# Mamo1031/Multimodal-MTRSSM

Measured on AMD Instinct MI355X. Metric: seq-steps/s (BxT) MoPoE-MRSSM train step, higher is better.
Workload: dtype bf16x2-split, fp32 accumulate; 1 GPU; BASELINE configs[1]: MoPoE-MRSSM train step, B=64/GPU T=50 deter=200 stoch=30, vision 1x64x64 + audio 1x128x32 + action 4; global_batch=64, seq_len=50, parallelism=dp1, hidden=200, embed=256, categoricals_x_classes=6x5, residual_blocks=3, activation=ELU, optimizer=AdamW lr 1e-3 + clip 10 (fused HIP), params=4151600, streams=1, launch=eager (host enqueues every launch), backend=none, rccl_ranks=0, collective_ranks=0, noise=uniforms keyed by global batch row (parallel.GlobalRowNoise)

## Files before the change

multimodal_mtrssm_amd/csrc/mrssm_cluster.hip:

```cpp
#include "scan_common.h"

namespace mtrssm {

void set_error(const char* fmt, ...);
void set_last_kernel(const char* name);
int device_cu_count();

constexpr int kClu = 4;
constexpr int kCluThreads = 256;
constexpr unsigned kSpinLimit = 1u << 22;

__device__ unsigned long long* g_cluster_prof = nullptr;
#define MTRSSM_CLU_STAMP(i)                                                                                  \
  do {                                                                                                       \
    if (prof && t >= 8 && t < 12) prof[(t - 8) * 16 + (i)] = __builtin_readcyclecounter();                   \
  } while (0)

__device__ __forceinline__ void granule_store(unsigned long long* p, unsigned epoch, float v) {
  __hip_atomic_store(p, ((unsigned long long)epoch << 32) | (unsigned long long)__float_as_uint(v), __ATOMIC_RELAXED,
                     __HIP_MEMORY_SCOPE_AGENT);
}

template <int NJ>
__device__ __forceinline__ bool wave_gather(const unsigned long long* g, float* dst, int total, unsigned epoch, int lane) {
  unsigned done = 0;
  const unsigned full = (1u << NJ) - 1u;
#pragma unroll
  for (int j = 0; j < NJ; ++j)
    if (lane + 64 * j >= total) done |= 1u << j;
  for (unsigned spins = 0;; ++spins) {
#pragma unroll
    for (int j = 0; j < NJ; ++j) {
      if (!(done & (1u << j))) {
        const unsigned long long x = __hip_atomic_load(g + lane + 64 * j, __ATOMIC_RELAXED, __HIP_MEMORY_SCOPE_AGENT);
        if ((unsigned)(x >> 32) == epoch) {
          dst[lane + 64 * j] = __uint_as_float((unsigned)x);
          done |= 1u << j;
        }
      }
    }
    if (__all(done == full)) return true;
    if (spins > kSpinLimit) return false;
    __builtin_amdgcn_s_sleep(1);
  }
}

template <int DH, int NP, int PPT, bool MASKED>
__global__ __launch_bounds__(kCluThreads) void mrssm_fwd_cluster_kernel(const MtrssmMrssmDims dm, const MtrssmMrssmClusterWeights w,
                                                                        const MtrssmMrssmFwdIO io, unsigned long long* __restrict__ gran,
                                                                        int* __restrict__ status, int nclusters) {
  extern __shared__ __attribute__((aligned(16))) float lds[];
  constexpr int D = DH, H = DH;
  constexpr int UD = D / kClu, UH = H / kClu;
  constexpr int NG = 3 * UD, NH = 3 * UH;
  constexpr int KP = DH / NP;
  constexpr int NPIECE = 2 * NG * NP;
  static_assert(KP % 4 == 0 && DH % NP == 0, "pieces are whole float4 runs");
  static_assert(PPT * kCluThreads >= NPIECE, "every piece has a thread");
  const int K = dm.K, C = dm.C, S = K * C, T = dm.T, act = dm.act;
  const int tid = threadIdx.x, lane = tid & (kWave - 1), wave = tid / kWave;
  const int blk = blockIdx.x;
  const int member = (blk >> 3) & (kClu - 1);
  const int cluster = (blk & 7) + 8 * (blk >> 5);
  if (cluster >= nclusters) return;

  int o = 0;
  auto take = [&](int n) { const int r = o; o += (n + 3) & ~3; return r; };
  const int Ls = take(S), Lh1 = take(DH), Ld0 = take(DH), Ld1 = take(DH), Lhd = take(3 * 64);
  const int Llp = take(S), Lla = take(S), Llv = take(S), Lmx = take(S);
  const int Lpart = take(kClu * 3 * S);
  const int Lred = take(NPIECE > NH * NP ? NPIECE : NH * NP);
  const int Lw1 = take(S * H);
  const int Lwh = take(D * NH);
  const int Lbl = take(3 * S);
  const int Lu = take(2 * 64);
  const int Lflag = take(4);
  (void)o;
  int* abort_flag = reinterpret_cast<int*>(lds + Lflag);

  float wreg[PPT][KP];
  int xsel[PPT];
#pragma unroll
  for (int i = 0; i < PPT; ++i) {
    const int pc = tid * PPT + i;
    const int pcc = pc < NPIECE ? pc : NPIECE - 1;
    const int col = pcc / NP, part = pcc - col * NP;
    const bool is_h = col >= NG;
    const int og = is_h ? col - NG : col;
    const int gcol = (og / UD) * D + member * UD + (og % UD);
    const float* src = (is_h ? w.whh_t : w.wf_t) + (size_t)(part * KP) * 3 * D + gcol;
    xsel[i] = (is_h ? 1 : 0) | (part * KP) << 1;
#pragma unroll
    for (int k = 0; k < KP; ++k) wreg[i][k] = src[(size_t)k * 3 * D];
  }
  float wrow[64];
  {
    const bool roleL = tid < 3 * S;
    const int which = roleL ? tid / S : 0, srow = roleL ? tid - which * S : 0;
    const float* rowsrc = (which == 0 ? w.w4 : (which == 1 ? w.wa2 : w.wv2)) + (size_t)srow * H + member * UH;
#pragma unroll
    for (int k = 0; k < 64; ++k) wrow[k] = k < UH ? rowsrc[k] : 0.f;
  }
  for (int idx = tid; idx < S * H; idx += kCluThreads) lds[Lw1 + idx] = w.w1s_t[idx];
  for (int idx = tid; idx < D * NH; idx += kCluThreads) {
    const int k = idx / NH, oh = idx - k * NH;
    lds[Lwh + idx] = w.wh1_t[(size_t)k * 3 * H + (oh / UH) * H + member * UH + (oh % UH)];
  }
  for (int i = tid; i < 3 * 64; i += kCluThreads) lds[Lhd + i] = 0.f;
  for (int i = tid; i < 3 * S; i += kCluThreads) {
    const int which = i / S, s2 = i - which * S;
    lds[Lbl + i] = (which == 0 ? w.b4 : (which == 1 ? w.ba2 : w.bv2))[s2];
  }
  float bias_g[6] = {0.f, 0.f, 0.f, 0.f, 0.f, 0.f};
  if (tid < UD) {
#pragma unroll
    for (int g = 0; g < 3; ++g) {
      bias_g[g] = w.bf[g * D + member * UD + tid];
      bias_g[3 + g] = w.bhh[g * D + member * UD + tid];
    }
  }
  const float bias_h = (tid < UH) ? w.b3[member * UH + tid] : 0.f;
  if (tid == 0) *abort_flag = 0;

  const int slotsD = UD, slotsL = 3 * S;
  const int per_parity = kClu * (slotsD + slotsL);
  unsigned long long* gbase = gran + (size_t)cluster * 2 * per_parity;
  unsigned epoch = 0;
  unsigned long long* prof = (blockIdx.x == 0 && tid == 0) ? g_cluster_prof : nullptr;

  for (int row = cluster; row < dm.B; row += nclusters) {
    int cur = Ld0, nxt = Ld1;
    lds_barrier();
    for (int i = tid; i < D; i += kCluThreads) lds[cur + i] = io.deter0[(size_t)row * D + i];
    for (int i = tid; i < S; i += kCluThreads) lds[Ls + i] = io.stoch0[(size_t)row * S + i];
    lds_barrier();

    auto load_inputs = [&](size_t q, float& xa_r, float& pa_r, float& up_r, float& ur_r, int& code_r) {
      code_r = modality_code<MASKED>(io.modality, q);
      xa_r = tid < H ? io.xa[q * H + tid] : 0.f;
      pa_r = 0.f;
      if (tid >= UH && tid < NH) {
        const int which = tid / UH, u = tid - which * UH;
        pa_r = (which == 1 ? io.pa : io.pv)[q * H + member * UH + u];
      }
      up_r = (wave == 3 && lane < K) ? io.u_post[q * K + lane] : 0.f;
      ur_r = (wave == 3 && lane < K && io.u_prior) ? io.u_prior[q * K + lane] : 0.f;
    };
    float xa_n, pav_n, up_n, ur_n;
    int code_n;
    load_inputs((size_t)row * T, xa_n, pav_n, up_n, ur_n, code_n);

    for (int t = 0; t < T; ++t) {
      const size_t bt = (size_t)row * T + t;
      unsigned long long* gpar = gbase + (size_t)(t & 1) * per_parity;
      const float xa_v = xa_n, pav = pav_n;
      const int code = code_n;
      if (wave == 3 && lane < K) { lds[Lu + lane] = up_n; lds[Lu + 64 + lane] = ur_n; }
      if (t + 1 < T) load_inputs(bt + 1, xa_n, pav_n, up_n, ur_n, code_n);

      MTRSSM_CLU_STAMP(0);
      if (tid < H) {
        const float* wc = lds + Lw1 + tid;
        float a0 = xa_v, a1 = 0.f, a2 = 0.f, a3 = 0.f;
        int k = 0;
        for (; k + 8 <= S; k += 8) {
          float wv[8], sv[8];
#pragma unroll
          for (int i = 0; i < 8; ++i) { wv[i] = wc[(size_t)(k + i) * H]; sv[i] = lds[Ls + k + i]; }
          a0 = fmaf(wv[0], sv[0], a0); a1 = fmaf(wv[1], sv[1], a1); a2 = fmaf(wv[2], sv[2], a2); a3 = fmaf(wv[3], sv[3], a3);
          a0 = fmaf(wv[4], sv[4], a0); a1 = fmaf(wv[5], sv[5], a1); a2 = fmaf(wv[6], sv[6], a2); a3 = fmaf(wv[7], sv[7], a3);
        }
        for (; k < S; ++k) a0 = fmaf(wc[(size_t)k * H], lds[Ls + k], a0);
        const float h = act_fwd((a0 + a1) + (a2 + a3), act);
        lds[Lh1 + tid] = h;
        if (member == 0 && io.sv_h1) io.sv_h1[bt * H + tid] = h;
      }
      lds_barrier();

      MTRSSM_CLU_STAMP(1);
#pragma unroll
      for (int i = 0; i < PPT; ++i) {
        const float* xv = lds + ((xsel[i] & 1) ? cur : Lh1) + (xsel[i] >> 1);
        float a0 = 0.f, a1 = 0.f, a2 = 0.f, a3 = 0.f;
#pragma unroll
        for (int k = 0; k < KP; k += 4) {
          const float4 x = *reinterpret_cast<const float4*>(xv + k);
          a0 = fmaf(wreg[i][k], x.x, a0);
          a1 = fmaf(wreg[i][k + 1], x.y, a1);
          a2 = fmaf(wreg[i][k + 2], x.z, a2);
          a3 = fmaf(wreg[i][k + 3], x.w, a3);
        }
        if (tid * PPT + i < NPIECE) lds[Lred + tid * PPT + i] = (a0 + a1) + (a2 + a3);
      }
      lds_barrier();

      MTRSSM_CLU_STAMP(2);
      ++epoch;
      if (tid < UD) {
        float gs[6];
#pragma unroll
        for (int g = 0; g < 6; ++g) {
          const float* pr = lds + Lred + ((g < 3 ? g : g - 3) * UD + tid + (g < 3 ? 0 : NG)) * NP;
          float a = bias_g[g];
#pragma unroll
          for (int q = 0; q < NP; ++q) a += pr[q];
          gs[g] = a;
        }
        const float rg = __fdividef(1.f, 1.f + __expf(-(gs[3] + gs[0])));
        const float zg = __fdividef(1.f, 1.f + __expf(-(gs[4] + gs[1])));
        const float ng = 1.f - __fdividef(2.f, __expf(2.f * (gs[2] + gs[5] * rg)) + 1.f);
        const int unit = member * UD + tid;
        const float dnew = (lds[cur + unit] - ng) * zg + ng;
        lds[nxt + unit] = dnew;
        granule_store(gpar + (size_t)member * slotsD + tid, epoch, dnew);
        io.deter[bt * D + unit] = dnew;
        if (io.sv_gates) {
          float* gsv = io.sv_gates + bt * 4 * D;
          gsv[unit] = rg; gsv[D + unit] = zg; gsv[2 * D + unit] = ng; gsv[3 * D + unit] = gs[5];
        }
      }
      if (wave == 3) {
        const bool ok = wave_gather<4>(gpar, lds + nxt, D, epoch, lane);
        if (!ok && lane == 0) { *abort_flag = 1; atomicExch(status, 1 + 2 * t); }
      }
      lds_barrier();
// ... 35 lines not shown
      if (tid < 3 * S) {
        const float* hv = lds + Lhd + (tid / S) * 64;
        float p0 = 0.f, p1 = 0.f;
#pragma unroll
        for (int u = 0; u < 64; u += 4) {
          const float4 x = *reinterpret_cast<const float4*>(hv + u);
          p0 = fmaf(wrow[u], x.x, p0);
          p1 = fmaf(wrow[u + 1], x.y, p1);
          p0 = fmaf(wrow[u + 2], x.z, p0);
          p1 = fmaf(wrow[u + 3], x.w, p1);
        }
        const float p = p0 + p1;
        lds[Lpart + member * 3 * S + tid] = p;
        granule_store(gl + (size_t)member * slotsL + tid, epoch, p);
      }
      if (wave == 3) {
        const bool ok = wave_gather<6>(gl, lds + Lpart, kClu * 3 * S, epoch, lane);
        if (!ok && lane == 0) { *abort_flag = 1; atomicExch(status, 2 + 2 * t); }
      }
      lds_barrier();
      if (*abort_flag) return;

      MTRSSM_CLU_STAMP(5);
      if (wave == 3) {
        const bool writer = member == 0;
        for (int i = lane; i < 3 * S; i += kWave) {
          const int which = i / S, s2 = i - which * S;
          float v = lds[Lbl + i];
#pragma unroll
          for (int m2 = 0; m2 < kClu; ++m2) v += lds[Lpart + m2 * 3 * S + i];
          lds[(which == 0 ? Llp : (which == 1 ? Lla : Llv)) + s2] = v;
        }
        wave_mopoe_mix_masked<true, MASKED>(lds + Lla, lds + Llv, lds + Llp, lds + Lmx, S, lane, code);
        for (int s = lane; s < S; s += kWave) {
          if (writer) {
            io.prior_logits[bt * S + s] = lds[Llp + s];
            io.post_logits[bt * S + s] = lds[Lmx + s];
            if (io.sv_la) { io.sv_la[bt * S + s] = lds[Lla + s]; io.sv_lv[bt * S + s] = lds[Llv + s]; }
          }
        }
        float kl = C <= 8 ? cat_block_fwd_fast8(lds + Lmx, lds + Llp, K, C, lane, lds + Lu, io.u_prior ? lds + Lu + 64 : nullptr, lds + Ls,
                                                io.post_stoch + bt * S, io.prior_stoch ? io.prior_stoch + bt * S : nullptr, writer)
                          : cat_block_fwd<true, true>(lds + Lmx, lds + Llp, K, C, lane, lds + Lu, io.u_prior ? lds + Lu + 64 : nullptr, lds + Ls,
                                                      io.post_stoch + bt * S, io.prior_stoch ? io.prior_stoch + bt * S : nullptr, writer);
        if (io.kl) {
          kl = wave_sum(kl);
          if (lane == 0 && writer) io.kl[bt] = kl;
        }
      }
      lds_barrier();
      MTRSSM_CLU_STAMP(7);
      const int tmp = cur; cur = nxt; nxt = tmp;
    }
  }
}

template <int NJ, typename Map>
__device__ __forceinline__ bool wave_gather_map(int total, unsigned epoch, int lane, Map map) {
  unsigned done = 0;
  const unsigned full = (1u << NJ) - 1u;
#pragma unroll
  for (int j = 0; j < NJ; ++j)
    if (lane + 64 * j >= total) done |= 1u << j;
  for (unsigned spins = 0;; ++spins) {
#pragma unroll
    for (int j = 0; j < NJ; ++j) {
      if (!(done & (1u << j))) {
        const unsigned long long* slot;
        float* dst;
        map(lane + 64 * j, slot, dst);
        const unsigned long long x = __hip_atomic_load(slot, __ATOMIC_RELAXED, __HIP_MEMORY_SCOPE_AGENT);
// ... 25 lines not shown
  static_assert(NG % NPB == 0 && KPB % 2 == 0, "row pieces are whole float2 runs");
  static_assert(PPT * kCluThreads >= NPIECE, "every row piece has a thread");
  const int K = dm.K, C = dm.C, S = K * C, T = dm.T, act = dm.act;
  const int tid = threadIdx.x, lane = tid & (kWave - 1), wave = tid / kWave;
  const int blk = blockIdx.x;
  const int member = (blk >> 3) & (kClu - 1);
  const int cluster = (blk & 7) + 8 * (blk >> 5);
  if (cluster >= nclusters) return;

  int o = 0;
  auto take = [&](int n) { const int r = o; o += (n + 3) & ~3; return r; };
  const int Lla = take(S), Llv = take(S), Lmx = take(S), Llp = take(S), Ldmx = take(S), Ldlp = take(S), Ldla = take(S), Ldlv = take(S);
  const int Lgps = take(S), Lcs = take(S);
  const int Lhd = take(NHP), Ldzh = take(NHP);
  const int Lgate = take(4 * UD), Ldprev = take(UD), Lgd = take(UD), Lcd = take(UD);
  const int Ldg = take(2 * NG);
  const int Lh1 = take(DH), Ldz1 = take(DH);
  const int Lpdd = take(kClu * UD);
  const int Lpcd = take(kClu * UD), Lpdh = take(kClu * DH);
  const int Lred = take(NPIECE > DH ? NPIECE : DH);
  const int Lred2 = take(W1P * 64 > 3 * 64 ? W1P * 64 : 3 * 64);
  const int Lwh = take(D * NHP);
  const int Lw2 = take(32 * NHP);
  const int Lflag = take(4);
  (void)o;
  int* abort_flag = reinterpret_cast<int*>(lds + Lflag);
  float* gk_lds = lds + Lflag + 1;

  float wreg[PPT][KPB];
#pragma unroll
  for (int i = 0; i < PPT; ++i) {
    const int pc = tid * PPT + i;
    const int pcc = pc < NPIECE ? pc : NPIECE - 1;
    const int rowi = pcc / NPB, part = pcc - rowi * NPB;
    const bool is_f = rowi >= DH;
    const float* src = (is_f ? w.wf_t : w.whh_t) + (size_t)(is_f ? rowi - DH : rowi) * 3 * D;
#pragma unroll
    for (int k = 0; k < KPB; ++k) {
      const int og = part * KPB + k;
      wreg[i][k] = src[(og / UD) * D + member * UD + (og % UD)];
    }
  }
  for (int idx = tid; idx < 32 * NHP; idx += kCluThreads) {
    const int s2 = idx / NHP, j = idx - s2 * NHP;
    float v = 0.f;
    if (s2 < S && j < NH) {
// ... 1 lines not shown
      v = (which == 0 ? w.w4 : (which == 1 ? w.wa2 : w.wv2))[(size_t)s2 * H + member * UH + u];
    }
    lds[Lw2 + idx] = v;
  }
  float w1r[KW1];
  {
    const int srow = tid / W1P < S ? tid / W1P : 0, part = tid % W1P;
#pragma unroll
    for (int k = 0; k < KW1; ++k) {
      const int kk = part * KW1 + k;
      w1r[k] = w.w1s_t[(size_t)srow * H + (kk < H ? kk : H - 1)];
    }
  }
  for (int idx = tid; idx < D * NHP; idx += kCluThreads) {
    const int k = idx / NHP, oh = idx - k * NHP;
    lds[Lwh + idx] = oh < NH ? w.wh1_t[(size_t)k * 3 * H + (oh / UH) * H + member * UH + (oh % UH)] : 0.f;
  }
  for (int i = tid; i < NHP; i += kCluThreads) { lds[Lhd + i] = 0.f; lds[Ldzh + i] = 0.f; }
  if (tid == 0) *abort_flag = 0;

  const int per_parity = kClu * 3 * D;
  unsigned long long* gbase = gran + (size_t)cluster * 2 * per_parity;
  unsigned epoch = 0;

  for (int row = cluster; row < dm.B; row += nclusters) {
    lds_barrier();
    for (int i = tid; i < UD; i += kCluThreads) lds[Lcd + i] = 0.f;
    for (int i = tid; i < S; i += kCluThreads) lds[Lcs + i] = 0.f;
    lds_barrier();

    float r0 = 0.f, r1 = 0.f, r2 = 0.f, r3 = 0.f, r4 = 0.f;
    int code_n = kModBoth;
    auto stage_load = [&](int tt) {
      const size_t q = (size_t)row * T + tt;
      code_n = modality_code<MASKED>(io.modality, q);
      if (tid < 4 * S) {
        const int which = tid / S, s2 = tid - which * S;
        const float* src = which == 0 ? io.sv_la : (which == 1 ? io.sv_lv : (which == 2 ? io.post_logits : io.prior_logits));
        r0 = src[q * S + s2];
      }
      if (tid < NH) {
        const int which = tid / UH, u = tid - which * UH;
        r1 = io.sv_heads[q * 3 * H + which * H + member * UH + u];
      } else if (tid < NH + S) {
        r1 = io.g_post_stoch ? io.g_post_stoch[q * S + (tid - NH)] : 0.f;
      }
// ... 10 lines not shown
      } else if (tid >= 64 && tid < 64 + UD) {
        r4 = io.g_deter ? io.g_deter[q * D + member * UD + (tid - 64)] : 0.f;
      }
    };
    auto stage_store = [&]() {
      if (tid < 4 * S) {
        const int which = tid / S, s2 = tid - which * S;
        lds[(which == 0 ? Lla : (which == 1 ? Llv : (which == 2 ? Lmx : Llp))) + s2] = r0;
      }
      if (tid < NH) lds[Lhd + tid] = r1;
      else if (tid < NH + S) lds[Lgps + tid - NH] = r1;
      if (tid < 4 * UD) lds[Lgate + tid] = r2;
      else if (tid == 4 * UD) *gk_lds = r2;
      if (tid < H) lds[Lh1 + tid] = r3;
      if (tid < UD) lds[Ldprev + tid] = r4;
      else if (tid >= 64 && tid < 64 + UD) lds[Lgd + tid - 64] = r4;
    };
    stage_load(T - 1);

    for (int t = T - 1; t >= 0; --t) {
      const size_t bt = (size_t)row * T + t;
      unsigned long long* gpar = gbase + (size_t)(t & 1) * per_parity;

      stage_store();
      const int code = code_n;
      if (t > 0) stage_load(t - 1);
      lds_barrier();

      if (wave == 3) {
        if (C <= 8)
          cat_block_bwd_fast8(lds + Lmx, lds + Llp, K, C, lane, lds + Lgps, lds + Lcs, io.g_prior_stoch ? io.g_prior_stoch + bt * S : nullptr,
                              io.g_post_logits ? io.g_post_logits + bt * S : nullptr, io.g_prior_logits ? io.g_prior_logits + bt * S : nullptr,
                              *gk_lds, dm.kl_w_post, dm.kl_w_prior, lds + Ldmx, lds + Ldlp);
        else
          cat_block_bwd<true>(lds + Lmx, lds + Llp, K, C, lane, lds + Lgps, lds + Lcs, io.g_prior_stoch ? io.g_prior_stoch + bt * S : nullptr,
                              io.g_post_logits ? io.g_post_logits + bt * S : nullptr, io.g_prior_logits ? io.g_prior_logits + bt * S : nullptr,
                              *gk_lds, dm.kl_w_post, dm.kl_w_prior, lds + Ldmx, lds + Ldlp);
        wave_mopoe_mix_bwd_masked<true, MASKED>(lds + Lla, lds + Llv, lds + Lmx, lds + Ldmx, lds + Ldla, lds + Ldlv, lds + Ldlp, S, lane,
                                                code);
        if (member == 0) {
          for (int s2 = lane; s2 < S; s2 += kWave) {
            io.d_la[bt * S + s2] = lds[Ldla + s2];
            io.d_lv[bt * S + s2] = lds[Ldlv + s2];
            io.d_lp[bt * S + s2] = lds[Ldlp + s2];
          }
        }
      }
      lds_barrier();

      if (tid < NH) {
        const int which = tid / UH;
        const float* dl = lds + (which == 0 ? Ldlp : (which == 1 ? Ldla : Ldlv));
        const float* wc2 = lds + Lw2 + tid;
        float a0 = 0.f, a1 = 0.f;
#pragma unroll
        for (int s2 = 0; s2 < 32; s2 += 2) {
          a0 = fmaf(wc2[s2 * NHP], s2 < S ? dl[s2] : 0.f, a0);
          a1 = fmaf(wc2[(s2 + 1) * NHP], s2 + 1 < S ? dl[s2 + 1] : 0.f, a1);
        }
        const float g = (a0 + a1) * act_grad_from_out(lds[Lhd + tid], act);
        lds[Ldzh + tid] = g;
        const int u = tid - which * UH;
        io.d_zh[bt * 3 * H + which * H + member * UH + u] = g;
      }
      lds_barrier();

      ++epoch;
      if (tid < D) {
        const float* wr = lds + Lwh + (size_t)tid * NHP;
        const float* dz = lds + Ldzh;
        float p0 = 0.f, p1 = 0.f, p2 = 0.f, p3 = 0.f;
#pragma unroll
        for (int j = 0; j < NHP; j += 4) {
          const float4 a = *reinterpret_cast<const float4*>(wr + j);
          const float4 b = *reinterpret_cast<const float4*>(dz + j);
          p0 = fmaf(a.x, b.x, p0); p1 = fmaf(a.y, b.y, p1); p2 = fmaf(a.z, b.z, p2); p3 = fmaf(a.w, b.w, p3);
        }
        granule_store(gpar + (size_t)member * D + tid, epoch, (p0 + p1) + (p2 + p3));
      }
      if (wave == 3) {
        const bool ok = wave_gather_map<4>(kClu * UD, epoch, lane, [&](int i, const unsigned long long*& slot, float*& dst) {
          const int m2 = i / UD, u = i - m2 * UD;
          slot = gpar + (size_t)m2 * D + member * UD + u;
          dst = lds + Lpdd + i;
        });
        if (!ok && lane == 0) { *abort_flag = 1; atomicExch(status, 1 + 2 * t); }
      }
      lds_barrier();
      if (*abort_flag) return;

      if (tid < UD) {
        float dd = lds[Lgd + tid] + lds[Lcd + tid];
#pragma unroll
        for (int m2 = 0; m2 < kClu; ++m2) dd += lds[Lpdd + m2 * UD + tid];
        const float rg = lds[Lgate + tid], zg = lds[Lgate + UD + tid], ng = lds[Lgate + 2 * UD + tid], ghn = lds[Lgate + 3 * UD + tid];
        const float dprev = lds[Ldprev + tid];
        const float dn = dd * (1.f - zg);
        const float dz = dd * (dprev - ng);
        const float dn_pre = dn * (1.f - ng * ng);
        const float dr = dn_pre * ghn;
        const float dr_pre = dr * rg * (1.f - rg);
        const float dz_pre = dz * zg * (1.f - zg);
        lds[Lcd + tid] = dd * zg;
        lds[Ldg + tid] = dr_pre; lds[Ldg + UD + tid] = dz_pre; lds[Ldg + 2 * UD + tid] = dn_pre;
        lds[Ldg + NG + tid] = dr_pre; lds[Ldg + NG + UD + tid] = dz_pre; lds[Ldg + NG + 2 * UD + tid] = dn_pre * rg;
        const int unit = member * UD + tid;
        float* gi = io.d_gi + bt * 3 * D;
        float* gh = io.d_gh + bt * 3 * D;
        gi[unit] = dr_pre; gi[D + unit] = dz_pre; gi[2 * D + unit] = dn_pre;
        gh[unit] = dr_pre; gh[D + unit] = dz_pre; gh[2 * D + unit] = dn_pre * rg;
      }
      lds_barrier();

#pragma unroll
      for (int i = 0; i < PPT; ++i) {
        const int pc = tid * PPT + i;
        const int pcc = pc < NPIECE ? pc : NPIECE - 1;
        const int rowi = pcc / NPB, part = pcc - rowi * NPB;
        const float* xv = lds + Ldg + (rowi >= DH ? 0 : NG) + part * KPB;
        float a0 = 0.f, a1 = 0.f;
#pragma unroll
        for (int k = 0; k < KPB; k += 2) {
          const float2 x = *reinterpret_cast<const float2*>(xv + k);
          a0 = fmaf(wreg[i][k], x.x, a0);
          a1 = fmaf(wreg[i][k + 1], x.y, a1);
        }
        if (pc < NPIECE) lds[Lred + pc] = a0 + a1;
      }
      lds_barrier();
      ++epoch;
      unsigned long long* g2 = gpar + (size_t)kClu * D;
      for (int r2 = tid; r2 < 2 * DH; r2 += kCluThreads) {
        float a = 0.f;
#pragma unroll
        for (int q = 0; q < NPB; ++q) a += lds[Lred + r2 * NPB + q];
        granule_store(g2 + (size_t)member * 2 * D + r2, epoch, a);
      }
      if (wave >= 1) {
        bool ok;
        if (wave == 1) {
          ok = wave_gather_map<4>(kClu * UD, epoch, lane, [&](int i, const unsigned long long*& slot, float*& dst) {
            const int m2 = i / UD, u = i - m2 * UD;
            slot = g2 + (size_t)m2 * 2 * D + member * UD + u;
            dst = lds + Lpcd + i;
          });
        } else {
          const int mb = (wave - 2) * 2;
          ok = wave_gather_map<(2 * DH + 63) / 64>(2 * DH, epoch, lane, [&](int i, const unsigned long long*& slot, float*& dst) {
            const int m2 = mb + i / DH, k = i % DH;
            slot = g2 + (size_t)m2 * 2 * D + D + k;
            dst = lds + Lpdh + m2 * DH + k;
          });
        }
        if (!ok && lane == 0) { *abort_flag = 1; atomicExch(status, 2 + 2 * t); }
      }
      lds_barrier();
      if (*abort_flag) return;

      if (tid < UD) {
        float a = lds[Lcd + tid];
#pragma unroll
        for (int m2 = 0; m2 < kClu; ++m2) a += lds[Lpcd + m2 * UD + tid];
        lds[Lcd + tid] = a;
      }
      if (tid < H) {
        float a = 0.f;
#pragma unroll
        for (int m2 = 0; m2 < kClu; ++m2) a += lds[Lpdh + m2 * DH + tid];
        const float g = a * act_grad_from_out(lds[Lh1 + tid], act);
        lds[Ldz1 + tid] = g;
        if (member == 0) io.d_z1[bt * H + tid] = g;
      }
      lds_barrier();
      {
        const int srow = tid / W1P, part = tid % W1P;
        if (srow < S) {
          float a0 = 0.f;
#pragma unroll
          for (int k = 0; k < KW1; ++k) {
            const int kk = part * KW1 + k;
            a0 = fmaf(w1r[k], kk < H ? lds[Ldz1 + kk] : 0.f, a0);
          }
          lds[Lred2 + srow * W1P + part] = a0;
        }
      }
      lds_barrier();
      if (tid < S) {
        float a = 0.f;
#pragma unroll
        for (int q = 0; q < W1P; ++q) a += lds[Lred2 + tid * W1P + q];
        lds[Lcs + tid] = a;
      }
      lds_barrier();
    }
    if (tid < UD) io.g_deter0[(size_t)row * D + member * UD + tid] = lds[Lcd + tid];
    if (member == 0 && tid < S) io.g_stoch0[(size_t)row * S + tid] = lds[Lcs + tid];
  }
}

static int cluster_npb(int DH) { return (DH == 200 || DH == 128) ? 3 : 1; }

static size_t cluster_bwd_lds_floats(int DH, int S) {
  const int UD = DH / kClu, NG = 3 * UD, NH = NG, NHP = (NH + 3) & ~3, NPB = cluster_npb(DH), NPIECE = 2 * DH * NPB;
  size_t o = 0;
  auto take = [&](size_t n) { o += (n + 3) & ~(size_t)3; };
  for (int i = 0; i < 10; ++i) take(S);
  take(NHP); take(NHP);
  take((size_t)4 * UD); take(UD); take(UD); take(UD);
  take((size_t)2 * NG);
  take(DH); take(DH);
  take((size_t)kClu * UD);
  take((size_t)kClu * UD); take((size_t)kClu * DH);
  take((size_t)(NPIECE > DH ? NPIECE : DH));
  take((size_t)(8 * 64));
  take((size_t)DH * NHP);
  take((size_t)32 * NHP);
  take(4);
  return o;
}

size_t mrssm_cluster_bwd_workspace_bytes(const MtrssmMrssmDims* d) {
  if (!d || d->B <= 0 || d->D <= 0) return 0;
  const int nclusters = d->B < 64 ? d->B : 64;
  return 16 + (size_t)nclusters * 2 * (size_t)kClu * 3 * d->D * sizeof(unsigned long long);
}

int mrssm_cluster_supported(const MtrssmMrssmDims* d);

int mrssm_bwd_cluster_launch(const MtrssmMrssmDims* d, const MtrssmMrssmClusterWeights* w, const MtrssmMrssmBwdIO* io, void* workspace,
                             size_t workspace_bytes, hipStream_t stream) {
  if (!mrssm_cluster_supported(d) || d->K * d->C > 32) {
    set_error("mrssm_rollout_bwd_cluster: dims outside the cluster kernel's regime (ask mtrssm_mrssm_cluster_supported first; S <= 32)");
    return MTRSSM_EINVAL;
  }
  if (!w || !io || !workspace || !w->w1s_t || !w->wf_t || !w->whh_t || !w->wh1_t || !w->w4 || !w->wa2 || !w->wv2 || !io->deter0 ||
      !io->deter || !io->prior_logits || !io->post_logits || !io->sv_h1 || !io->sv_gates || !io->sv_heads || !io->sv_la || !io->sv_lv ||
      !io->g_deter0 || !io->g_stoch0 || !io->d_z1 || !io->d_gi || !io->d_gh || !io->d_zh || !io->d_lp || !io->d_la || !io->d_lv) {
    set_error("mrssm_rollout_bwd_cluster: null required pointer");
    return MTRSSM_EINVAL;
// ... 32 lines not shown
#undef MTRSSM_CLUB_LAUNCH
#undef MTRSSM_CLUB_LAUNCH_M
  e = hipGetLastError();
  if (e != hipSuccess) { set_error("cluster backward scan launch failed: %s", hipGetErrorString(e)); return MTRSSM_ELAUNCH; }
  return MTRSSM_OK;
}

int debug_set_cluster_profile(void* buf) {
  unsigned long long* p = static_cast<unsigned long long*>(buf);
  return hipMemcpyToSymbol(HIP_SYMBOL(g_cluster_prof), &p, sizeof(p)) == hipSuccess ? MTRSSM_OK : MTRSSM_ELAUNCH;
}

static int cluster_kw(int D, int H) { return D > H ? D : H; }

static int cluster_np(int DH) { return DH == 200 ? 5 : (DH == 128 ? 4 : (DH == 64 ? 2 : 1)); }

static size_t cluster_lds_floats(int D, int H, int S) {
  const int UD = D / kClu, UH = H / kClu, NG = 3 * UD, NH = 3 * UH, KW = cluster_kw(D, H), NP = cluster_np(KW);
  size_t o = 0;
  auto take = [&](size_t n) { o += (n + 3) & ~(size_t)3; };
  take(S); take(KW); take(KW); take(KW); take(3 * 64);
  take(S); take(S); take(S); take(S);
  take((size_t)kClu * 3 * S);
  take((size_t)(2 * NG * NP > NH * NP ? 2 * NG * NP : NH * NP));
  take((size_t)S * H);
  take((size_t)D * NH);
  take((size_t)3 * S);
  take(2 * 64);
  take(4);
  return o;
}

size_t mrssm_cluster_workspace_bytes(const MtrssmMrssmDims* d) {
  if (!d || d->B <= 0 || d->D <= 0 || d->K <= 0 || d->C <= 0) return 0;
  const int nclusters = d->B < 64 ? d->B : 64;
  const size_t per_parity = (size_t)kClu * (d->D / kClu + 3 * d->K * d->C);
  return 16 + (size_t)nclusters * 2 * per_parity * sizeof(unsigned long long);
}

int mrssm_cluster_supported(const MtrssmMrssmDims* d) {
  if (!d || d->B <= 0 || d->T <= 0 || d->D <= 0 || d->H <= 0 || d->K <= 0 || d->C <= 0 || !d->post) return 0;
  const int S = d->K * d->C, D = d->D, H = d->H;
  if (D != H || (D != 32 && D != 64 && D != 128 && D != 200)) return 0;
  if (3 * S > kCluThreads || H / kClu > 64 || 3 * H / kClu > kCluThreads || d->K > 64) return 0;
  if (D > 4 * kWave || kClu * 3 * S > 6 * kWave) return 0;
  if (cluster_lds_floats(D, H, S) * sizeof(float) > 160 * 1024) return 0;
  const int nclusters = d->B < 64 ? d->B : 64;
  if (device_cu_count() < ((nclusters + 7) / 8) * 32) return 0;
  return 1;
}

// ... 19 lines not shown
  const int grid = groups * 32;
  const size_t lds = cluster_lds_floats(d->D, d->H, d->K * d->C) * sizeof(float);
  if (int rc = clear_async(static_cast<char*>(workspace) + 16, mrssm_cluster_workspace_bytes(d) - 16, stream)) return rc;
  hipError_t e = hipSuccess;
  int* status = reinterpret_cast<int*>(workspace);
  unsigned long long* gran = reinterpret_cast<unsigned long long*>(reinterpret_cast<char*>(workspace) + 16);
  const int kw = cluster_kw(d->D, d->H);
#define MTRSSM_CLU_LAUNCH_M(DHV, NPV, PPTV, MV)                                                                                     \
  {                                                                                                                               \
    e = hipFuncSetAttribute(reinterpret_cast<const void*>(mrssm_fwd_cluster_kernel<DHV, NPV, PPTV, MV>),                          \
                            hipFuncAttributeMaxDynamicSharedMemorySize, (int)lds);                                               \
    if (e != hipSuccess) { set_error("hipFuncSetAttribute(max dynamic LDS=%zu): %s", lds, hipGetErrorString(e)); return MTRSSM_ELAUNCH; } \
    set_last_kernel("mtrssm::mrssm_fwd_cluster_kernel<" #DHV ", " #NPV ", " #PPTV ", " #MV ">");                                 \
    hipLaunchKernelGGL((mrssm_fwd_cluster_kernel<DHV, NPV, PPTV, MV>), dim3(grid), dim3(kCluThreads), lds, stream, *d, *w, *io,     \
                       gran, status, nclusters);                                                                                  \
  }
#define MTRSSM_CLU_LAUNCH(DHV, NPV, PPTV)                      \
  {                                                           \
    if (io->modality) MTRSSM_CLU_LAUNCH_M(DHV, NPV, PPTV, true) \
    else MTRSSM_CLU_LAUNCH_M(DHV, NPV, PPTV, false)             \
  }
  if (kw == 32) MTRSSM_CLU_LAUNCH(32, 1, 1)
  else if (kw == 64) MTRSSM_CLU_LAUNCH(64, 2, 1)
  else if (kw == 128) MTRSSM_CLU_LAUNCH(128, 4, 3)
  else MTRSSM_CLU_LAUNCH(200, 5, 6)
#undef MTRSSM_CLU_LAUNCH
#undef MTRSSM_CLU_LAUNCH_M
  e = hipGetLastError();
  if (e != hipSuccess) { set_error("cluster scan launch failed: %s", hipGetErrorString(e)); return MTRSSM_ELAUNCH; }
  return MTRSSM_OK;
}

}
```

multimodal_mtrssm_amd/csrc/scan_common.h:

```cpp
#pragma once
#include <hip/hip_runtime.h>
#include <stdint.h>

#include "../../include/mtrssm.h"

namespace mtrssm {

constexpr int kWave = 64;

int clear_async(void* p, size_t bytes, hipStream_t stream);
constexpr float kLogThird = -1.0986122886681098f;

__device__ __forceinline__ float act_fwd(float z, int act) {
  switch (act) {
    case MTRSSM_ACT_RELU: return z > 0.f ? z : 0.f;
    case MTRSSM_ACT_ELU: return z > 0.f ? z : expm1f(z);
    case MTRSSM_ACT_TANH: return tanhf(z);
    default: return z;
  }
}

__device__ __forceinline__ float act_grad_from_out(float h, int act) {
  switch (act) {
    case MTRSSM_ACT_RELU: return h > 0.f ? 1.f : 0.f;
// ... 279 lines not shown
    for (int c = 0; c < 8; ++c)
      if (c < C) klk += eq[c] * rq * (((q[c] - qm) - lqs) - ((p[c] - pm) - lps));
    kl += klk;
    const float u = u_post[k];
    float acc = 0.f;
    int idx = 0;
#pragma unroll
    for (int c = 0; c < 7; ++c)
      if (c + 1 < C) { acc += eq[c] * rq; idx += (acc <= u) ? 1 : 0; }
#pragma unroll
    for (int c = 0; c < 8; ++c)
      if (c < C) {
        const float v = c == idx ? 1.f : 0.f;
        s_lds[k * C + c] = v;
        if (ok) post_stoch_g[k * C + c] = v;
      }
    if (u_prior && prior_stoch_g && ok) {
      const float up = u_prior[k];
      float pacc = 0.f;
      int pidx = 0;
#pragma unroll
      for (int c = 0; c < 7; ++c)
        if (c + 1 < C) { pacc += ep[c] * rp; pidx += (pacc <= up) ? 1 : 0; }
#pragma unroll
      for (int c = 0; c < 8; ++c)
        if (c < C) prior_stoch_g[k * C + c] = c == pidx ? 1.f : 0.f;
    }
  }
  return kl;
}

template <bool FAST = false>
__device__ __forceinline__ void cat_block_bwd(const float* q_logits, const float* p_logits, int K, int C, int lane,
                                              const float* g_post_stoch, const float* carry_s,
                                              const float* g_prior_stoch, const float* g_post_logits,
                                              const float* g_prior_logits, float gk, float w_post, float w_prior,
                                              float* dq, float* dp) {
  for (int k = lane; k < K; k += kWave) {
    const float* ql = q_logits + k * C;
    const float* pl = p_logits + k * C;
    float qm, qs, pm, ps;
    cat_stats<FAST>(ql, C, qm, qs);
    cat_stats<FAST>(pl, C, pm, ps);
    const float lqs = clog<FAST>(qs), lps = clog<FAST>(ps);
    const float rq = 1.f / qs, rp = 1.f / ps;
    float dot = 0.f, klk = 0.f, pdot = 0.f;
// ... 82 lines not shown
  wave_flat_lse<FAST>(lv, S, lane, mv, lsv);
  float suma = 0.f, sumv = 0.f;
  for (int s = lane; s < S; s += kWave) {
    const float a = (la[s] - ma) - lsa;
    const float v = (lv[s] - mv) - lsv;
    const float mx = mixed[s];
    const float wa = cexp<FAST>(kLogThird + a - mx), wv = cexp<FAST>(kLogThird + v - mx), wf = cexp<FAST>(kLogThird + a + v - mx);
    const float g = dmx[s];
    const float da = g * (wa + wf), dv = g * (wv + wf);
    dla[s] = da;
    dlv[s] = dv;
    suma += da;
    sumv += dv;
  }
  suma = wave_sum(suma);
  sumv = wave_sum(sumv);
  for (int s = lane; s < S; s += kWave) {
    dla[s] -= cexp<FAST>((la[s] - ma) - lsa) * suma;
    dlv[s] -= cexp<FAST>((lv[s] - mv) - lsv) * sumv;
  }
}

template <bool FAST, bool MASKED>
__device__ __forceinline__ void wave_mopoe_mix_bwd_masked(const float* la, const float* lv, const float* mixed, const float* dmx,
                                                          float* dla, float* dlv, float* dlp, int S, int lane, int code) {
  if (!MASKED || code == kModBoth) {
    wave_mopoe_mix_bwd<FAST>(la, lv, mixed, dmx, dla, dlv, S, lane);
    return;
  }
  if (code == 0) {
    for (int s = lane; s < S; s += kWave) {
      dlp[s] += dmx[s];
      dla[s] = 0.f;
      dlv[s] = 0.f;
    }
    return;
  }
  const float* l = code == 1 ? la : lv;
  float* dl = code == 1 ? dla : dlv;
  float* dz = code == 1 ? dlv : dla;
  float m, ls;
  wave_flat_lse<FAST>(l, S, lane, m, ls);
  float sum = 0.f;
  for (int s = lane; s < S; s += kWave) {
    sum += dmx[s];
    dz[s] = 0.f;
// ... 17 lines not shown
```

Before: 364,400 seq-steps/s.

## Overlap recurrent h-gate matvec and split MoPoE/categorical work across waves

The forward cluster kernel now keeps separate register weights for the input and recurrent GRU matvecs and computes the recurrent part for the next step (gh_pieces) on idle waves while waves 0-2 compute LSE and prior statistics in parallel. Wave 3 then finishes the mix and sampling from those precomputed stats. The first matvec exploits the one-hot stochastic state by gathering only the selected weight columns via stored sample indices. The backward kernel splits the mix gradient into a coefficient phase on wave 0, overlapped with the categorical backward, and a finish phase, and gains profiling stamps. In exchange it adds LDS buffers, extra barriers and more register pressure from doubled weight registers.

```diff
diff --git a/multimodal_mtrssm_amd/csrc/mrssm_cluster.hip b/multimodal_mtrssm_amd/csrc/mrssm_cluster.hip
--- a/multimodal_mtrssm_amd/csrc/mrssm_cluster.hip
+++ b/multimodal_mtrssm_amd/csrc/mrssm_cluster.hip
@@ -45,7 +45,7 @@
   }
 }
 
-template <int DH, int NP, int PPT, bool MASKED>
+template <int DH, int NP, int PH, bool MASKED>
 __global__ __launch_bounds__(kCluThreads) void mrssm_fwd_cluster_kernel(const MtrssmMrssmDims dm, const MtrssmMrssmClusterWeights w,
                                                                         const MtrssmMrssmFwdIO io, unsigned long long* __restrict__ gran,
                                                                         int* __restrict__ status, int nclusters) {
@@ -54,9 +54,9 @@
   constexpr int UD = D / kClu, UH = H / kClu;
   constexpr int NG = 3 * UD, NH = 3 * UH;
   constexpr int KP = DH / NP;
-  constexpr int NPIECE = 2 * NG * NP;
+  constexpr int NPK = NG * NP;
   static_assert(KP % 4 == 0 && DH % NP == 0, "pieces are whole float4 runs");
-  static_assert(PPT * kCluThreads >= NPIECE, "every piece has a thread");
+  static_assert(PH * kCluThreads >= NPK, "every piece has a thread");
   const int K = dm.K, C = dm.C, S = K * C, T = dm.T, act = dm.act;
   const int tid = threadIdx.x, lane = tid & (kWave - 1), wave = tid / kWave;
   const int blk = blockIdx.x;
@@ -69,30 +69,49 @@
   const int Ls = take(S), Lh1 = take(DH), Ld0 = take(DH), Ld1 = take(DH), Lhd = take(3 * 64);
   const int Llp = take(S), Lla = take(S), Llv = take(S), Lmx = take(S);
   const int Lpart = take(kClu * 3 * S);
-  const int Lred = take(NPIECE > NH * NP ? NPIECE : NH * NP);
+  const int Lred = take(NPK);
+  const int Lgh = take(NPK);
   const int Lw1 = take(S * H);
   const int Lwh = take(D * NH);
   const int Lbl = take(3 * S);
   const int Lu = take(2 * 64);
+  const int Lst = take(4 * 64 + S);
+  const int Lidx = take(64);
   const int Lflag = take(4);
   (void)o;
   int* abort_flag = reinterpret_cast<int*>(lds + Lflag);
-
-  float wreg[PPT][KP];
-  int xsel[PPT];
-#pragma unroll
-  for (int i = 0; i < PPT; ++i) {
-    const int pc = tid * PPT + i;
-    const int pcc = pc < NPIECE ? pc : NPIECE - 1;
-    const int col = pcc / NP, part = pcc - col * NP;
-    const bool is_h = col >= NG;
-    const int og = is_h ? col - NG : col;
+  int* sidx = reinterpret_cast<int*>(lds + Lidx);
+
+  float wreg[PH][KP], wregh[PH][KP];
+  int xoff[PH];
+#pragma unroll
+  for (int i = 0; i < PH; ++i) {
+    const int pc = tid * PH + i;
+    const int pcc = pc < NPK ? pc : NPK - 1;
+    const int og = pcc / NP, part = pcc - og * NP;
     const int gcol = (og / UD) * D + member * UD + (og % UD);
-    const float* src = (is_h ? w.whh_t : w.wf_t) + (size_t)(part * KP) * 3 * D + gcol;
-    xsel[i] = (is_h ? 1 : 0) | (part * KP) << 1;
-#pragma unroll
-    for (int k = 0; k < KP; ++k) wreg[i][k] = src[(size_t)k * 3 * D];
-  }
+    const float* srci = w.wf_t + (size_t)(part * KP) * 3 * D + gcol;
+    const float* srch = w.whh_t + (size_t)(part * KP) * 3 * D + gcol;
+    xoff[i] = part * KP;
+#pragma unroll
+    for (int k = 0; k < KP; ++k) { wreg[i][k] = srci[(size_t)k * 3 * D]; wregh[i][k] = srch[(size_t)k * 3 * D]; }
+  }
+  auto gh_pieces = [&](const float* dv) {
+#pragma unroll
+    for (int i = 0; i < PH; ++i) {
+      const float* xv = dv + xoff[i];
+      float a0 = 0.f, a1 = 0.f, a2 = 0.f, a3 = 0.f;
+#pragma unroll
+      for (int k = 0; k < KP; k += 4) {
+        const float4 x = *reinterpret_cast<const float4*>(xv + k);
+        a0 = fmaf(wregh[i][k], x.x, a0);
+        a1 = fmaf(wregh[i][k + 1], x.y, a1);
+        a2 = fmaf(wregh[i][k + 2], x.z, a2);
+        a3 = fmaf(wregh[i][k + 3], x.w, a3);
+      }
+      if (tid * PH + i < NPK) lds[Lgh + tid * PH + i] = (a0 + a1) + (a2 + a3);
+    }
+  };
   float wrow[64];
   {
     const bool roleL = tid < 3 * S;
@@ -134,6 +153,7 @@
     for (int i = tid; i < D; i += kCluThreads) lds[cur + i] = io.deter0[(size_t)row * D + i];
     for (int i = tid; i < S; i += kCluThreads) lds[Ls + i] = io.stoch0[(size_t)row * S + i];
     lds_barrier();
+    gh_pieces(lds + cur);
 
     auto load_inputs = [&](size_t q, float& xa_r, float& pa_r, float& up_r, float& ur_r, int& code_r) {
       code_r = modality_code<MASKED>(io.modality, q);
@@ -163,6 +183,28 @@
         const float* wc = lds + Lw1 + tid;
         float a0 = xa_v, a1 = 0.f, a2 = 0.f, a3 = 0.f;
         int k = 0;
+        if (t > 0 && C <= 8) {
+          const int s8 = S & ~7;
+          for (int kb = 0; kb < K; kb += 8) {
+            float wv[8];
+            int ch[8];
+#pragma unroll
+            for (int i = 0; i < 8; ++i) {
+              const int kk = kb + i < K ? kb + i : K - 1;
+              const int sel = kk * C + sidx[kk];
+              wv[i] = wc[(size_t)sel * H];
+              ch[i] = kb + i < K ? (sel < s8 ? (sel & 3) : 0) : 4;
+            }
+#pragma unroll
+            for (int i = 0; i < 8; ++i) {
+              a0 = ch[i] == 0 ? fmaf(wv[i], 1.f, a0) : a0;
+              a1 = ch[i] == 1 ? fmaf(wv[i], 1.f, a1) : a1;
+              a2 = ch[i] == 2 ? fmaf(wv[i], 1.f, a2) : a2;
+              a3 = ch[i] == 3 ? fmaf(wv[i], 1.f, a3) : a3;
+            }
+          }
+          k = S;
+        }
         for (; k + 8 <= S; k += 8) {
           float wv[8], sv[8];
 #pragma unroll
@@ -179,8 +221,8 @@
 
       MTRSSM_CLU_STAMP(1);
 #pragma unroll
-      for (int i = 0; i < PPT; ++i) {
-        const float* xv = lds + ((xsel[i] & 1) ? cur : Lh1) + (xsel[i] >> 1);
+      for (int i = 0; i < PH; ++i) {
+        const float* xv = lds + Lh1 + xoff[i];
         float a0 = 0.f, a1 = 0.f, a2 = 0.f, a3 = 0.f;
 #pragma unroll
         for (int k = 0; k < KP; k += 4) {
@@ -190,7 +232,7 @@
           a2 = fmaf(wreg[i][k + 2], x.z, a2);
           a3 = fmaf(wreg[i][k + 3], x.w, a3);
         }
-        if (tid * PPT + i < NPIECE) lds[Lred + tid * PPT + i] = (a0 + a1) + (a2 + a3);
+        if (tid * PH + i < NPK) lds[Lred + tid * PH + i] = (a0 + a1) + (a2 + a3);
       }
       lds_barrier();
 
@@ -200,7 +242,7 @@
         float gs[6];
 #pragma unroll
         for (int g = 0; g < 6; ++g) {
-          const float* pr = lds + Lred + ((g < 3 ? g : g - 3) * UD + tid + (g < 3 ? 0 : NG)) * NP;
+          const float* pr = lds + (g < 3 ? Lred : Lgh) + ((g < 3 ? g : g - 3) * UD + tid) * NP;
           float a = bias_g[g];
 #pragma unroll
           for (int q = 0; q < NP; ++q) a += pr[q];
@@ -282,31 +324,57 @@
       if (*abort_flag) return;
 
       MTRSSM_CLU_STAMP(5);
+      const bool writer = member == 0;
+      const bool fast8 = C <= 8;
+      if (tid < 3 * S) {
+        const int which = tid / S, s2 = tid - which * S;
+        float v = lds[Lbl + tid];
+#pragma unroll
+        for (int m2 = 0; m2 < kClu; ++m2) v += lds[Lpart + m2 * 3 * S + tid];
+        lds[(which == 0 ? Llp : (which == 1 ? Lla : Llv)) + s2] = v;
+      }
+      lds_barrier();
+      MTRSSM_CLU_STAMP(8);
+      if (wave == 0) {
+        if (code & 1) {
+          float m, ls;
+          wave_flat_lse<true>(lds + Lla, S, lane, m, ls);
+          if (lane == 0) { lds[Lst] = m; lds[Lst + 1] = ls; }
+        }
+        if (writer && io.sv_la)
+          for (int s = lane; s < S; s += kWave) io.sv_la[bt * S + s] = lds[Lla + s];
+      } else if (wave == 1) {
+        if (code & 2) {
+          float m, ls;
+          wave_flat_lse<true>(lds + Llv, S, lane, m, ls);
+          if (lane == 0) { lds[Lst + 2] = m; lds[Lst + 3] = ls; }
+        }
+        if (writer && io.sv_la)
+          for (int s = lane; s < S; s += kWave) io.sv_lv[bt * S + s] = lds[Llv + s];
+      } else if (wave == 2) {
+        if (fast8) cat_prior_stats_fast8(lds + Llp, K, C, lane, lds + Lst + 64, lds + Lst + 128, lds + Lst + 192, lds + Lst + 256);
+        if (writer)
+          for (int s = lane; s < S; s += kWave) io.prior_logits[bt * S + s] = lds[Llp + s];
+      } else if (t + 1 < T) {
+        gh_pieces(lds + nxt);
+      }
+      lds_barrier();
+      MTRSSM_CLU_STAMP(6);
       if (wave == 3) {
-        const bool writer = member == 0;
-        for (int i = lane; i < 3 * S; i += kWave) {
-          const int which = i / S, s2 = i - which * S;
-          float v = lds[Lbl + i];
-#pragma unroll
-          for (int m2 = 0; m2 < kClu; ++m2) v += lds[Lpart + m2 * 3 * S + i];
-          lds[(which == 0 ? Llp : (which == 1 ? Lla : Llv)) + s2] = v;
-        }
-        wave_mopoe_mix_masked<true, MASKED>(lds + Lla, lds + Llv, lds + Llp, lds + Lmx, S, lane, code);
-        for (int s = lane; s < S; s += kWave) {
-          if (writer) {
-            io.prior_logits[bt * S + s] = lds[Llp + s];
-            io.post_logits[bt * S + s] = lds[Lmx + s];
-            if (io.sv_la) { io.sv_la[bt * S + s] = lds[Lla + s]; io.sv_lv[bt * S + s] = lds[Llv + s]; }
-          }
-        }
-        float kl = C <= 8 ? cat_block_fwd_fast8(lds + Lmx, lds + Llp, K, C, lane, lds + Lu, io.u_prior ? lds + Lu + 64 : nullptr, lds + Ls,
-                                                io.post_stoch + bt * S, io.prior_stoch ? io.prior_stoch + bt * S : nullptr, writer)
-                          : cat_block_fwd<true, true>(lds + Lmx, lds + Llp, K, C, lane, lds + Lu, io.u_prior ? lds + Lu + 64 : nullptr, lds + Ls,
-                                                      io.post_stoch + bt * S, io.prior_stoch ? io.prior_stoch + bt * S : nullptr, writer);
+        wave_mopoe_mix_pre<true, MASKED>(lds + Lla, lds + Llv, lds + Llp, lds + Lst, lds + Lmx, S, lane, code);
+        if (writer)
+          for (int s = lane; s < S; s += kWave) io.post_logits[bt * S + s] = lds[Lmx + s];
+        float kl = fast8 ? cat_block_fwd_fast8_pre(lds + Lmx, lds + Llp, lds + Lst + 64, lds + Lst + 128, lds + Lst + 192, lds + Lst + 256, K, C,
+                                                   lane, lds + Lu, io.u_prior ? lds + Lu + 64 : nullptr, lds + Ls, sidx, io.post_stoch + bt * S,
+                                                   io.prior_stoch ? io.prior_stoch + bt * S : nullptr, writer)
+                         : cat_block_fwd<true, true>(lds + Lmx, lds + Llp, K, C, lane, lds + Lu, io.u_prior ? lds + Lu + 64 : nullptr, lds + Ls,
+                                                     io.post_stoch + bt * S, io.prior_stoch ? io.prior_stoch + bt * S : nullptr, writer);
         if (io.kl) {
           kl = wave_sum(kl);
           if (lane == 0 && writer) io.kl[bt] = kl;
         }
+      } else if (t + 1 < T) {
+        gh_pieces(lds + nxt);
       }
       lds_barrier();
       MTRSSM_CLU_STAMP(7);
@@ -378,6 +446,7 @@
   const int Lred2 = take(W1P * 64 > 3 * 64 ? W1P * 64 : 3 * 64);
   const int Lwh = take(D * NHP);
   const int Lw2 = take(32 * NHP);
+  const int Lca = take(S), Lcv = take(S), Lpa = take(S), Lpv = take(S);
   const int Lflag = take(4);
   (void)o;
   int* abort_flag = reinterpret_cast<int*>(lds + Lflag);
@@ -425,6 +494,7 @@
   const int per_parity = kClu * 3 * D;
   unsigned long long* gbase = gran + (size_t)cluster * 2 * per_parity;
   unsigned epoch = 0;
+  unsigned long long* prof = (blockIdx.x == 0 && tid == 0) ? g_cluster_prof : nullptr;
 
   for (int row = cluster; row < dm.B; row += nclusters) {
     lds_barrier();
@@ -481,11 +551,15 @@
       const size_t bt = (size_t)row * T + t;
       unsigned long long* gpar = gbase + (size_t)(t & 1) * per_parity;
 
+      MTRSSM_CLU_STAMP(0);
       stage_store();
       const int code = code_n;
       if (t > 0) stage_load(t - 1);
       lds_barrier();
 
+      MTRSSM_CLU_STAMP(1);
+      if (wave == 0)
+        wave_mopoe_mix_bwd_coef<true, MASKED>(lds + Lla, lds + Llv, lds + Lmx, lds + Lca, lds + Lcv, lds + Lpa, lds + Lpv, S, lane, code);
       if (wave == 3) {
         if (C <= 8)
           cat_block_bwd_fast8(lds + Lmx, lds + Llp, K, C, lane, lds + Lgps, lds + Lcs, io.g_prior_stoch ? io.g_prior_stoch + bt * S : nullptr,
@@ -495,8 +569,12 @@
           cat_block_bwd<true>(lds + Lmx, lds + Llp, K, C, lane, lds + Lgps, lds + Lcs, io.g_prior_stoch ? io.g_prior_stoch + bt * S : nullptr,
                               io.g_post_logits ? io.g_post_logits + bt * S : nullptr, io.g_prior_logits ? io.g_prior_logits + bt * S : nullptr,
                               *gk_lds, dm.kl_w_post, dm.kl_w_prior, lds + Ldmx, lds + Ldlp);
-        wave_mopoe_mix_bwd_masked<true, MASKED>(lds + Lla, lds + Llv, lds + Lmx, lds + Ldmx, lds + Ldla, lds + Ldlv, lds + Ldlp, S, lane,
-                                                code);
+      }
+      lds_barrier();
+      MTRSSM_CLU_STAMP(11);
+      if (wave == 3) {
+        wave_mopoe_mix_bwd_fin<MASKED>(lds + Lca, lds + Lcv, lds + Lpa, lds + Lpv, lds + Ldmx, lds + Ldla, lds + Ldlv, lds + Ldlp, S, lane,
+                                       code);
         if (member == 0) {
           for (int s2 = lane; s2 < S; s2 += kWave) {
             io.d_la[bt * S + s2] = lds[Ldla + s2];
@@ -507,6 +585,7 @@
       }
       lds_barrier();
 
+      MTRSSM_CLU_STAMP(2);
       if (tid < NH) {
         const int which = tid / UH;
         const float* dl = lds + (which == 0 ? Ldlp : (which == 1 ? Ldla : Ldlv));
@@ -524,6 +603,7 @@
       }
       lds_barrier();
 
+      MTRSSM_CLU_STAMP(3);
       ++epoch;
       if (tid < D) {
         const float* wr = lds + Lwh + (size_t)tid * NHP;
@@ -548,6 +628,7 @@
       lds_barrier();
       if (*abort_flag) return;
 
+      MTRSSM_CLU_STAMP(4);
       if (tid < UD) {
         float dd = lds[Lgd + tid] + lds[Lcd + tid];
 #pragma unroll
@@ -571,6 +652,7 @@
       }
       lds_barrier();
 
+      MTRSSM_CLU_STAMP(5);
 #pragma unroll
       for (int i = 0; i < PPT; ++i) {
         const int pc = tid * PPT + i;
@@ -587,6 +669,7 @@
         if (pc < NPIECE) lds[Lred + pc] = a0 + a1;
       }
       lds_barrier();
+      MTRSSM_CLU_STAMP(6);
       ++epoch;
       unsigned long long* g2 = gpar + (size_t)kClu * D;
       for (int r2 = tid; r2 < 2 * DH; r2 += kCluThreads) {
@@ -616,6 +699,7 @@
       lds_barrier();
       if (*abort_flag) return;
 
+      MTRSSM_CLU_STAMP(7);
       if (tid < UD) {
         float a = lds[Lcd + tid];
 #pragma unroll
@@ -631,6 +715,7 @@
         if (member == 0) io.d_z1[bt * H + tid] = g;
       }
       lds_barrier();
+      MTRSSM_CLU_STAMP(8);
       {
         const int srow = tid / W1P, part = tid % W1P;
         if (srow < S) {
@@ -644,6 +729,7 @@
         }
       }
       lds_barrier();
+      MTRSSM_CLU_STAMP(9);
       if (tid < S) {
         float a = 0.f;
 #pragma unroll
@@ -651,6 +737,7 @@
         lds[Lcs + tid] = a;
       }
       lds_barrier();
+      MTRSSM_CLU_STAMP(10);
     }
     if (tid < UD) io.g_deter0[(size_t)row * D + member * UD + tid] = lds[Lcd + tid];
     if (member == 0 && tid < S) io.g_stoch0[(size_t)row * S + tid] = lds[Lcs + tid];
@@ -674,6 +761,7 @@
   take((size_t)(8 * 64));
   take((size_t)DH * NHP);
   take((size_t)32 * NHP);
+  for (int i = 0; i < 4; ++i) take(S);
   take(4);
   return o;
 }
@@ -752,11 +840,14 @@
   take(S); take(KW); take(KW); take(KW); take(3 * 64);
   take(S); take(S); take(S); take(S);
   take((size_t)kClu * 3 * S);
-  take((size_t)(2 * NG * NP > NH * NP ? 2 * NG * NP : NH * NP));
+  take((size_t)(NG * NP > NH * NP ? NG * NP : NH * NP));
+  take((size_t)NG * NP);
   take((size_t)S * H);
   take((size_t)D * NH);
   take((size_t)3 * S);
   take(2 * 64);
+  take((size_t)4 * 64 + S);
+  take(64);
   take(4);
   return o;
 }
@@ -822,8 +913,8 @@
   }
   if (kw == 32) MTRSSM_CLU_LAUNCH(32, 1, 1)
   else if (kw == 64) MTRSSM_CLU_LAUNCH(64, 2, 1)
-  else if (kw == 128) MTRSSM_CLU_LAUNCH(128, 4, 3)
-  else MTRSSM_CLU_LAUNCH(200, 5, 6)
+  else if (kw == 128) MTRSSM_CLU_LAUNCH(128, 4, 2)
+  else MTRSSM_CLU_LAUNCH(200, 5, 3)
 #undef MTRSSM_CLU_LAUNCH
 #undef MTRSSM_CLU_LAUNCH_M
   e = hipGetLastError();
diff --git a/multimodal_mtrssm_amd/csrc/scan_common.h b/multimodal_mtrssm_amd/csrc/scan_common.h
--- a/multimodal_mtrssm_amd/csrc/scan_common.h
+++ b/multimodal_mtrssm_amd/csrc/scan_common.h
@@ -325,6 +325,117 @@
 #pragma unroll
       for (int c = 0; c < 7; ++c)
         if (c + 1 < C) { pacc += ep[c] * rp; pidx += (pacc <= up) ? 1 : 0; }
+#pragma unroll
+      for (int c = 0; c < 8; ++c)
+        if (c < C) prior_stoch_g[k * C + c] = c == pidx ? 1.f : 0.f;
+    }
+  }
+  return kl;
+}
+
+
+template <bool FAST, bool MASKED>
+__device__ __forceinline__ void wave_mopoe_mix_pre(const float* la, const float* lv, const float* lp, const float* lse, float* mixed,
+                                                   int S, int lane, int code) {
+  if (!MASKED || code == kModBoth) {
+    const float ma = lse[0], lsa = lse[1], mv = lse[2], lsv = lse[3];
+    for (int s = lane; s < S; s += kWave) {
+      const float a = (la[s] - ma) - lsa;
+      const float v = (lv[s] - mv) - lsv;
+      const float f = a + v;
+      const float x1 = kLogThird + a, x2 = kLogThird + v, x3 = kLogThird + f;
+      const float m = fmaxf(x1, fmaxf(x2, x3));
+      mixed[s] = clog<FAST>(cexp<FAST>(x1 - m) + cexp<FAST>(x2 - m) + cexp<FAST>(x3 - m)) + m;
+    }
+    return;
+  }
+  if (code == 0) {
+    for (int s = lane; s < S; s += kWave) mixed[s] = lp[s];
+    return;
+  }
+  const float* l = code == 1 ? la : lv;
+  const float m = code == 1 ? lse[0] : lse[2], ls = code == 1 ? lse[1] : lse[3];
+  for (int s = lane; s < S; s += kWave) mixed[s] = (l[s] - m) - ls;
+}
+
+__device__ __forceinline__ void cat_prior_stats_fast8(const float* p_logits, int K, int C, int lane, float* pm_o, float* lps_o, float* rp_o,
+                                                      float* ep_o) {
+  for (int k = lane; k < K; k += kWave) {
+    const float* pl = p_logits + k * C;
+    float p[8];
+#pragma unroll
+    for (int c = 0; c < 8; ++c) p[c] = c < C ? pl[c] : -INFINITY;
+    float pm = p[0];
+#pragma unroll
+    for (int c = 1; c < 8; ++c) pm = fmaxf(pm, p[c]);
+    float ep[8], ps = 0.f;
+#pragma unroll
+    for (int c = 0; c < 8; ++c) {
+      ep[c] = c < C ? __expf(p[c] - pm) : 0.f;
+      ps += ep[c];
+    }
+    pm_o[k] = pm;
+    lps_o[k] = __logf(ps);
+    rp_o[k] = __frcp_rn(ps);
+#pragma unroll
+    for (int c = 0; c < 8; ++c)
+      if (c < C) ep_o[k * C + c] = ep[c];
+  }
+}
+
+__device__ __forceinline__ float cat_block_fwd_fast8_pre(const float* q_logits, const float* p_logits, const float* pm_i, const float* lps_i,
+                                                         const float* rp_i, const float* ep_i, int K, int C, int lane, const float* u_post,
+                                                         const float* u_prior, float* s_lds, int* idx_o, float* post_stoch_g,
+                                                         float* prior_stoch_g, bool ok) {
+  float kl = 0.f;
+  for (int k = lane; k < K; k += kWave) {
+    const float* ql = q_logits + k * C;
+    const float* pl = p_logits + k * C;
+    float q[8], p[8];
+#pragma unroll
+    for (int c = 0; c < 8; ++c) {
+      q[c] = c < C ? ql[c] : -INFINITY;
+      p[c] = c < C ? pl[c] : -INFINITY;
+    }
+    const float pm = pm_i[k], lps = lps_i[k];
+    float qm = q[0];
+#pragma unroll
+    for (int c = 1; c < 8; ++c) qm = fmaxf(qm, q[c]);
+    float eq[8], qs = 0.f;
+#pragma unroll
+    for (int c = 0; c < 8; ++c) {
+      eq[c] = c < C ? __expf(q[c] - qm) : 0.f;
+      qs += eq[c];
+    }
+    const float rq = __frcp_rn(qs);
+    const float lqs = __logf(qs);
+    float klk = 0.f;
+#pragma unroll
+    for (int c = 0; c < 8; ++c)
+      if (c < C) klk += eq[c] * rq * (((q[c] - qm) - lqs) - ((p[c] - pm) - lps));
+    kl += klk;
+    const float u = u_post[k];
+    float acc = 0.f;
+    int idx = 0;
+#pragma unroll
+    for (int c = 0; c < 7; ++c)
+      if (c + 1 < C) { acc += eq[c] * rq; idx += (acc <= u) ? 1 : 0; }
+    idx_o[k] = idx;
+#pragma unroll
+    for (int c = 0; c < 8; ++c)
+      if (c < C) {
+        const float v = c == idx ? 1.f : 0.f;
+        s_lds[k * C + c] = v;
+        if (ok) post_stoch_g[k * C + c] = v;
+      }
+    if (u_prior && prior_stoch_g && ok) {
+      const float up = u_prior[k];
+      const float rp = rp_i[k];
+      float pacc = 0.f;
+      int pidx = 0;
+#pragma unroll
+      for (int c = 0; c < 7; ++c)
+        if (c + 1 < C) { pacc += ep_i[k * C + c] * rp; pidx += (pacc <= up) ? 1 : 0; }
 #pragma unroll
       for (int c = 0; c < 8; ++c)
         if (c < C) prior_stoch_g[k * C + c] = c == pidx ? 1.f : 0.f;
@@ -453,6 +564,74 @@
 }
 
 template <bool FAST, bool MASKED>
+__device__ __forceinline__ void wave_mopoe_mix_bwd_coef(const float* la, const float* lv, const float* mixed, float* ca, float* cv,
+                                                        float* pa, float* pv, int S, int lane, int code) {
+  if (!MASKED || code == kModBoth) {
+    float ma, lsa, mv, lsv;
+    wave_flat_lse<FAST>(la, S, lane, ma, lsa);
+    wave_flat_lse<FAST>(lv, S, lane, mv, lsv);
+    for (int s = lane; s < S; s += kWave) {
+      const float a = (la[s] - ma) - lsa;
+      const float v = (lv[s] - mv) - lsv;
+      const float mx = mixed[s];
+      const float wa = cexp<FAST>(kLogThird + a - mx), wv = cexp<FAST>(kLogThird + v - mx), wf = cexp<FAST>(kLogThird + a + v - mx);
+      ca[s] = wa + wf;
+      cv[s] = wv + wf;
+      pa[s] = cexp<FAST>((la[s] - ma) - lsa);
+      pv[s] = cexp<FAST>((lv[s] - mv) - lsv);
+    }
+    return;
+  }
+  if (code == 0) return;
+  const float* l = code == 1 ? la : lv;
+  float* pl = code == 1 ? pa : pv;
+  float m, ls;
+  wave_flat_lse<FAST>(l, S, lane, m, ls);
+  for (int s = lane; s < S; s += kWave) pl[s] = cexp<FAST>((l[s] - m) - ls);
+}
+
+template <bool MASKED>
+__device__ __forceinline__ void wave_mopoe_mix_bwd_fin(const float* ca, const float* cv, const float* pa, const float* pv, const float* dmx,
+                                                       float* dla, float* dlv, float* dlp, int S, int lane, int code) {
+  if (!MASKED || code == kModBoth) {
+    float suma = 0.f, sumv = 0.f;
+    for (int s = lane; s < S; s += kWave) {
+      const float g = dmx[s];
+      const float da = g * ca[s], dv = g * cv[s];
+      dla[s] = da;
+      dlv[s] = dv;
+      suma += da;
+      sumv += dv;
+    }
+    suma = wave_sum(suma);
+    sumv = wave_sum(sumv);
+    for (int s = lane; s < S; s += kWave) {
+      dla[s] -= pa[s] * suma;
+      dlv[s] -= pv[s] * sumv;
+    }
+    return;
+  }
+  if (code == 0) {
+    for (int s = lane; s < S; s += kWave) {
+      dlp[s] += dmx[s];
+      dla[s] = 0.f;
+      dlv[s] = 0.f;
+    }
+    return;
+  }
+  const float* pl = code == 1 ? pa : pv;
+  float* dl = code == 1 ? dla : dlv;
+  float* dz = code == 1 ? dlv : dla;
+  float sum = 0.f;
+  for (int s = lane; s < S; s += kWave) {
+    sum += dmx[s];
+    dz[s] = 0.f;
+  }
+  sum = wave_sum(sum);
+  for (int s = lane; s < S; s += kWave) dl[s] = dmx[s] - pl[s] * sum;
+}
+
+template <bool FAST, bool MASKED>
 __device__ __forceinline__ void wave_mopoe_mix_bwd_masked(const float* la, const float* lv, const float* mixed, const float* dmx,
                                                           float* dla, float* dlv, float* dlp, int S, int lane, int code) {
   if (!MASKED || code == kModBoth) {
```

Result: no change. 367,500 seq-steps/s (median of 6 runs) (+0.8%).
